# facebookresearch/DRTK

Hardware: AMD Instinct MI355X
Metric: Mpixels/sec fwd+bwd, 100k-tri @ 2048x2048, 1/2/4/8 GPU; HBM BW % (higher is better)
Workload: dtype f32; 1 GPU; 8 views/GPU x 1 GPU, 100k-tri UV-sphere head mesh (F=100352, V=50400), 2048x2048, C=16 attribute channels, transform+rasterize+render+interpolate+mask+edge_grad_estimator+loss fwd+bwd; views_per_gpu=8, triangles=100352, vertices=50400, height=2048, width=2048, channels=16, grad_reset=set_to_none, parallelism=single GPU

## Files before the change

drtk_amd/csrc/edge_grad.hip:

```cpp
#include <cstdlib>

#include "common.hpp"
#include "segscatter.hpp"

namespace drtk_amd {
namespace {

template <typename T>
struct Vec4;
template <>
struct Vec4<float> {
  using type = float4;
};
template <>
struct Vec4<double> {
  using type = double4;
};

template <typename T>
using Quad = T __attribute__((ext_vector_type(4), aligned(sizeof(T))));

template <typename T, int VEC>
struct Row {
  T v[VEC];
  T next;
};

template <typename T, int VEC>
__device__ __forceinline__ Row<T, VEC> load_row(
    const T* __restrict__ plane, int64_t row_off, int x, int W, bool x_ok, int lane) {
  Row<T, VEC> r;
  if (x_ok) {
    if constexpr (VEC == 4) {
      if (x + 4 <= W) {
        const Quad<T> q = *reinterpret_cast<const Quad<T>*>(plane + row_off + x);
        r.v[0] = q.x, r.v[1] = q.y, r.v[2] = q.z, r.v[3] = q.w;
      } else {
#pragma unroll
        for (int j = 0; j < 4; ++j) r.v[j] = x + j < W ? plane[row_off + x + j] : T(0);
      }
    } else {
      r.v[0] = plane[row_off + x];
    }
  } else {
#pragma unroll
    for (int j = 0; j < VEC; ++j) r.v[j] = T(0);
  }
  r.next = __shfl_down(r.v[0], 1);
  return r;
}

#ifndef DRTK_EDGE_SLOTS
#define DRTK_EDGE_SLOTS 64
#endif
#ifndef DRTK_ONEPASS_CAP
#define DRTK_ONEPASS_CAP 512
#endif
#ifndef DRTK_ONEPASS_WAVES
#define DRTK_ONEPASS_WAVES 6
#endif
constexpr int kOnepassCap = DRTK_ONEPASS_CAP;
#ifndef DRTK_EDGE_PRUNE
#define DRTK_EDGE_PRUNE 1
#endif

template <typename T>
struct PairArgs {
  const T* v_pix;
  const int32_t* vi;
  const T* bary_img;
  T* grad_v_pix;
  int64_t V, vi_sN;
  T M;
};

__device__ __forceinline__ int prefix4(int cnt, unsigned long long lt, int& total) {
  const unsigned long long b0 = __ballot(cnt & 1), b1 = __ballot(cnt & 2), b2 = __ballot(cnt & 4);
  total = __popcll(b0) + 2 * __popcll(b1) + 4 * __popcll(b2);
  return __popcll(b0 & lt) + 2 * __popcll(b1 & lt) + 4 * __popcll(b2 & lt);
}

template <typename T, int AXIS, int SLOTS>
__device__ __forceinline__ void scatter_pair_round(
    bool act, int px, int y, T term, const int32_t* __restrict__ idx_n, const T* __restrict__ v_n,
    const int32_t* __restrict__ vi_n, const T* __restrict__ bary_n, int64_t HW, int W, T M, int32_t* keys,
    TableAcc* vals, T* __restrict__ grad_n);

template <typename T, int R>
__device__ __forceinline__ uint32_t needed_pair_flags(
    uint32_t flags, int lane, int strip_x0, int y0, const int32_t* __restrict__ idx_n, const T* __restrict__ v_n,
    const int32_t* __restrict__ vi_n, int W, uint32_t* list, uint32_t* mask);

template <typename T, int VEC, int R, int WAVES, bool SCATTER = false>
__global__ __launch_bounds__(WAVES * kWave, SCATTER ? DRTK_ONEPASS_WAVES : 1) void edge_dots_kernel(
    const T* __restrict__ img, const T* __restrict__ grad_output, const int32_t* __restrict__ index_img, int C,
    int H, int W, int strips_x, T* __restrict__ gdx, T* __restrict__ gdy, int strip, T* __restrict__ zero_out,
    int64_t zero_count, PairArgs<T> pairs) {
  static_assert(!SCATTER || (VEC == 4 && 8 * R <= 32 && sizeof(T) == 4), "the pair phase works on four-pixel lanes of float; its flags are one register");
  constexpr int kSlots = DRTK_EDGE_SLOTS;
  constexpr int kCap = kOnepassCap;
  __shared__ uint2 s_list[SCATTER ? WAVES : 1][SCATTER ? kCap : 1];
  __shared__ int32_t t_keys[SCATTER ? WAVES : 1][SCATTER ? kSlots : 1];
  __shared__ TableAcc t_vals[SCATTER ? WAVES : 1][SCATTER ? kSlots * 4 : 1];
  if (zero_out) {
    const int64_t step = int64_t(gridDim.x) * gridDim.y * blockDim.x;
    for (int64_t i = (int64_t(blockIdx.y) * gridDim.x + blockIdx.x) * blockDim.x + threadIdx.x; i < zero_count; i += step) zero_out[i] = T(0);
  }
  const int64_t HW = int64_t(H) * W;
  const int n = blockIdx.y;
  const int tile = tile_index(strip);
  const int by = tile / strips_x, sx = tile - by * strips_x;
  const int lane = threadIdx.x & (kWave - 1);
  const int y0 = (by * WAVES + threadIdx.x / kWave) * R;
  if (y0 >= H) return;
  const int x = (sx * (kWave - 1) + lane) * VEC;
  const T* img_n = img + int64_t(n) * C * HW;
  const T* go_n = grad_output + int64_t(n) * C * HW;

  bool any_fg = false;
  uint32_t flags = 0;
  {
    const int32_t* idx_n = index_img + int64_t(n) * HW;
    int32_t above[4] = {-1, -1, -1, -1};
#pragma unroll
    for (int r = 0; r <= R; ++r) {
      const int y = y0 + r;
      if (y < H) {
        bool fg = false;
        int32_t first = -1, last = -1;
        int32_t cur[4] = {-1, -1, -1, -1};
        if (x < W) {
          if constexpr (VEC == 4) {
            Quad<int32_t> q;
            if (x + 4 <= W) {
              q = *reinterpret_cast<const Quad<int32_t>*>(idx_n + int64_t(y) * W + x);
            } else {
              const int32_t* rp = idx_n + int64_t(y) * W + x;
              q.x = rp[0], q.y = x + 1 < W ? rp[1] : -1, q.z = x + 2 < W ? rp[2] : -1, q.w = -1;
            }
            fg = (q.x & q.y & q.z & q.w) != -1;
            first = q.x, last = q.w;
            cur[0] = q.x, cur[1] = q.y, cur[2] = q.z, cur[3] = q.w;
          } else {
            first = last = idx_n[int64_t(y) * W + x];
            fg = first != -1;
          }
        }
        int32_t left = __shfl_up(last, 1), right = __shfl_down(first, 1);
        if (lane == 0) left = (x >= 1 && x < W) ? idx_n[int64_t(y) * W + x - 1] : -1;
        if (lane == kWave - 1) right = (x + VEC < W) ? idx_n[int64_t(y) * W + x + VEC] : -1;
        any_fg = any_fg || fg || left != -1 || right != -1;
        if constexpr (SCATTER) {
#pragma unroll
          for (int j = 0; j < 4; ++j) {
            const bool in_x = lane != kWave - 1 && x + j < W - 1;
            if (r > 0 && in_x && above[j] != cur[j]) flags |= 1u << (4 * R + 4 * (r - 1) + j);
            const int32_t nr = j < 3 ? cur[(j + 1) & 3] : right;
            if (r < R && in_x && y < H - 1 && cur[j] != nr) flags |= 1u << (4 * r + j);
            above[j] = cur[j];
          }
        }
      }
    }
  }
  bool load_any = any_fg;
  if constexpr (SCATTER) {
    if (__ballot(flags != 0) == 0) return;
#if DRTK_EDGE_PRUNE
    {
      static_assert(2 * kCap >= (kWave - 1) * 8 * R && kSlots >= kWave, "the list's storage must hold a strip's pair positions, the keys' one word per lane");
      const int wave = __builtin_amdgcn_readfirstlane(threadIdx.x / kWave);
      flags = needed_pair_flags<T, R>(
          flags, lane, sx * (kWave - 1) * VEC, y0, index_img + int64_t(n) * HW, pairs.v_pix + int64_t(n) * pairs.V * 3,
          pairs.vi + int64_t(n) * pairs.vi_sN, W, reinterpret_cast<uint32_t*>(s_list[wave]), reinterpret_cast<uint32_t*>(t_keys[wave]));
      if (__ballot(flags != 0) == 0) return;
    }
#endif
    uint32_t h3 = 0;
#pragma unroll
    for (int r = 0; r < R; ++r) h3 |= flags & (8u << (4 * r));
    const int left_h3 = __shfl_up(static_cast<int>(h3), 1);
    load_any = flags != 0 || (lane > 0 && left_h3 != 0);
  } else {
    if (__ballot(any_fg) == 0) return;
  }
  const bool x_ok = x < W && load_any;

  T ax[R][VEC], ay[R][VEC];
#pragma unroll
  for (int r = 0; r < R; ++r)
#pragma unroll
    for (int j = 0; j < VEC; ++j) ax[r][j] = ay[r][j] = T(0);

  for (int c = 0; c < C; ++c) {
    const T* ip = img_n + int64_t(c) * HW;
    const T* gp = go_n + int64_t(c) * HW;
    Row<T, VEC> ri[R + 1], rg[R + 1];
#pragma unroll
    for (int r = 0; r <= R; ++r) {
      const bool y_ok = (y0 + r) < H;
      ri[r] = load_row<T, VEC>(ip, int64_t(y0 + r) * W, x, W, x_ok && y_ok, lane);
      rg[r] = load_row<T, VEC>(gp, int64_t(y0 + r) * W, x, W, x_ok && y_ok, lane);
    }
#pragma unroll
    for (int r = 0; r < R; ++r) {
#pragma unroll
      for (int j = 0; j < VEC; ++j) {
        const T inext = (j + 1 < VEC) ? ri[r].v[(j + 1) % VEC] : ri[r].next;
        const T gnext = (j + 1 < VEC) ? rg[r].v[(j + 1) % VEC] : rg[r].next;
        ax[r][j] += (inext - ri[r].v[j]) * (T(0.5) * (gnext + rg[r].v[j]));
        ay[r][j] += (ri[r + 1].v[j] - ri[r].v[j]) * (T(0.5) * (rg[r + 1].v[j] + rg[r].v[j]));
      }
    }
  }
  if constexpr (SCATTER) {
    const int wave = __builtin_amdgcn_readfirstlane(threadIdx.x / kWave);
    const int32_t* idx_n = index_img + int64_t(n) * HW;
    const T* v_n = pairs.v_pix + int64_t(n) * pairs.V * 3;
    const int32_t* vi_n = pairs.vi + int64_t(n) * pairs.vi_sN;
    const T* bary_n = pairs.bary_img + int64_t(n) * 3 * HW;
    T* grad_n = pairs.grad_v_pix + int64_t(n) * pairs.V * 3;
    const int strip_x0 = sx * (kWave - 1) * VEC;

    table_init<kSlots>(t_keys[wave]);
    for (int i = lane; i < kSlots * 4; i += kWave) t_vals[wave][i] = 0;

    const unsigned long long lt = (1ull << lane) - 1ull;
    int grand = 0;
#pragma unroll
    for (int g = 0; g < 2 * R; ++g) {
      int t;
      prefix4(__popc((flags >> (4 * g)) & 15u), lt, t);
      grand += t;
    }
    if (grand <= kCap) {
      int n_h = 0, n_all = 0;
#pragma unroll
      for (int axis = 0; axis < 2; ++axis) {
#pragma unroll
        for (int r = 0; r < R; ++r) {
          const uint32_t f = (flags >> (4 * R * axis + 4 * r)) & 15u;
          int t;
          int pos = n_all + prefix4(__popc(f), lt, t);
          n_all += t;
#pragma unroll
          for (int j = 0; j < 4; ++j) {
            if (f & (1u << j)) s_list[wave][pos++] = make_uint2((r << 8) | (lane * 4 + j), __builtin_bit_cast(uint32_t, axis == 0 ? ax[r][j] : ay[r][j]));
          }
        }
        if (axis == 0) n_h = n_all;
      }
      wave_lds_sync();

      for (int axis = 0; axis < 2; ++axis) {
        const int l_begin = axis == 0 ? 0 : n_h, l_end = axis == 0 ? n_h : n_all;
        for (int t0 = l_begin; t0 < l_end; t0 += kWave) {
          const int t = t0 + lane;
          const bool act = t < l_end;
          int px = 0, y = 0;
          T term = T(0);
          if (act) {
            const uint2 entry = s_list[wave][t];
            y = y0 + static_cast<int>(entry.x >> 8);
            px = strip_x0 + static_cast<int>(entry.x & 255u);
            term = __builtin_bit_cast(float, entry.y);
          }
          if (axis == 0) {
            scatter_pair_round<T, 0, kSlots>(act, px, y, term, idx_n, v_n, vi_n, bary_n, HW, W, pairs.M, t_keys[wave], t_vals[wave], grad_n);
          } else {
            scatter_pair_round<T, 1, kSlots>(act, px, y, term, idx_n, v_n, vi_n, bary_n, HW, W, pairs.M, t_keys[wave], t_vals[wave], grad_n);
          }
        }
      }
    } else {
      static_assert(2 * kCap >= kWave * 8 * R, "the list's storage must hold a strip's terms");
      uint32_t* s_terms = reinterpret_cast<uint32_t*>(s_list[wave]);
#pragma unroll
      for (int q = 0; q < 4 * R; ++q) {
        s_terms[q * kWave + lane] = __builtin_bit_cast(uint32_t, ax[q / 4][q % 4]);
        s_terms[(4 * R + q) * kWave + lane] = __builtin_bit_cast(uint32_t, ay[q / 4][q % 4]);
      }
      wave_lds_sync();
      for (int axis = 0; axis < 2; ++axis) {
#pragma unroll 1
        for (int k = 0; k < 4 * R; ++k) {
          const bool act = (flags >> (4 * R * axis + k)) & 1u;
          if (__ballot(act) == 0) continue;
          const T term = __builtin_bit_cast(float, s_terms[(4 * R * axis + k) * kWave + lane]);
          if (axis == 0) {
            scatter_pair_round<T, 0, kSlots>(act, x + (k & 3), y0 + (k >> 2), term, idx_n, v_n, vi_n, bary_n, HW, W, pairs.M, t_keys[wave], t_vals[wave], grad_n);
          } else {
            scatter_pair_round<T, 1, kSlots>(act, x + (k & 3), y0 + (k >> 2), term, idx_n, v_n, vi_n, bary_n, HW, W, pairs.M, t_keys[wave], t_vals[wave], grad_n);
          }
        }
      }
    }
    wave_lds_sync();
    table_flush<T, TableAcc, kSlots>(t_keys[wave], t_vals[wave], 4, 3, grad_n, 3, 0);
    return;
  }
  if (!x_ok || lane == kWave - 1) return;
  T* ox = gdx + int64_t(n) * HW;
  T* oy = gdy + int64_t(n) * HW;
#pragma unroll
  for (int r = 0; r < R; ++r) {
    const int y = y0 + r;
    if (y >= H) break;
    const int64_t o = int64_t(y) * W + x;
    if constexpr (VEC == 4) {
      if (x + 4 <= W) {
        *reinterpret_cast<Quad<T>*>(ox + o) = Quad<T>{ax[r][0], ax[r][1], ax[r][2], ax[r][3]};
        *reinterpret_cast<Quad<T>*>(oy + o) = Quad<T>{ay[r][0], ay[r][1], ay[r][2], ay[r][3]};
      } else {
#pragma unroll
        for (int j = 0; j < 4; ++j)
          if (x + j < W) ox[o + j] = ax[r][j], oy[o + j] = ay[r][j];
      }
    } else {
      ox[o] = ax[r][0];
      oy[o] = ay[r][0];
    }
  }
}

template <typename T>
struct TriInfo {
  T p0x, p0y, p1x, p1y;
  T v01x, v01y, v02x, v02y, v12x, v12y;
  T den;
  T nx, ny, nz;
  int32_t i0, i1, i2;
};

template <typename T>
__device__ __forceinline__ void load_tri(
    const T* __restrict__ v_n, const int32_t* __restrict__ vi_n, int32_t idx, TriInfo<T>& t) {
  t.i0 = t.i1 = t.i2 = 0;
  if (idx >= 0) {
    const int32_t* f = vi_n + int64_t(idx) * 3;
    t.i0 = f[0], t.i1 = f[1], t.i2 = f[2];
  }
  t.p0x = v_n[3 * (int64_t)t.i0 + 0];
  t.p0y = v_n[3 * (int64_t)t.i0 + 1];
  t.p1x = v_n[3 * (int64_t)t.i1 + 0];
  t.p1y = v_n[3 * (int64_t)t.i1 + 1];
  const T p2x = v_n[3 * (int64_t)t.i2 + 0], p2y = v_n[3 * (int64_t)t.i2 + 1];
  t.v01x = t.p1x - t.p0x;
  t.v01y = t.p1y - t.p0y;
  t.v02x = p2x - t.p0x;
  t.v02y = p2y - t.p0y;
  t.v12x = p2x - t.p1x;
  t.v12y = p2y - t.p1y;
  t.den = t.v01x * t.v02y - t.v01y * t.v02x;
}

template <typename T>
__device__ __forceinline__ bool pix_in_tri(const TriInfo<T>& t, int x, int y) {
  if (t.den != T(0)) {
    const T px = static_cast<T>(x), py = static_cast<T>(y);
    const T vp0x = px - t.p0x, vp0y = py - t.p0y;
    const T vp1x = px - t.p1x, vp1y = py - t.p1y;
    T b0 = vp1y * t.v12x - vp1x * t.v12y;
    T b1 = vp0x * t.v02y - vp0y * t.v02x;
    T b2 = vp0y * t.v01x - vp0x * t.v01y;
    const T s = t.den > T(0) ? T(1) : (t.den < T(0) ? T(-1) : T(0));
    b0 *= s;
    b1 *= s;
    b2 *= s;
    const bool inside = (b0 >= T(0)) && (b1 >= T(0)) && (b2 >= T(0));
    const bool on0 = b0 == T(0), on1 = b1 == T(0), on2 = b2 == T(0);
    const bool pos = t.den > T(0);
    const bool tl0 = pos ? (t.v12y < T(0) || (t.v12y == T(0) && t.v12x > T(0)))
                         : (t.v12y > T(0) || (t.v12y == T(0) && t.v12x < T(0)));
    const bool tl1 = pos ? (t.v02y > T(0) || (t.v02y == T(0) && t.v02x < T(0)))
                         : (t.v02y < T(0) || (t.v02y == T(0) && t.v02x > T(0)));
    const bool tl2 = pos ? (t.v01y < T(0) || (t.v01y == T(0) && t.v01x > T(0)))
                         : (t.v01y > T(0) || (t.v01y == T(0) && t.v01x < T(0)));
    return inside && !((on0 && !tl0) || (on1 && !tl1) || (on2 && !tl2));
  }
  return false;
}

__device__ __forceinline__ float sqrt_t(float x) {
  return __builtin_sqrtf(x);
}
__device__ __forceinline__ double sqrt_t(double x) {
  return __builtin_sqrt(x);
}

template <typename T>
__device__ __forceinline__ void tri_normal(const T* __restrict__ v_n, TriInfo<T>& t) {
  const T* p0 = v_n + 3 * (int64_t)t.i0;
  const T* p1 = v_n + 3 * (int64_t)t.i1;
  const T* p2 = v_n + 3 * (int64_t)t.i2;
  const T ax = p0[0] - p2[0], ay = p0[1] - p2[1], az = p0[2] - p2[2];
  const T bx = p1[0] - p0[0], by = p1[1] - p0[1], bz = p1[2] - p0[2];
  const T cx = ay * bz - az * by;
  const T cy = az * bx - ax * bz;
  const T cz = ax * by - ay * bx;
  const T inv = T(1.0) / sqrt_t(cx * cx + cy * cy + cz * cz);
  t.nx = cx * inv;
  t.ny = cy * inv;
  t.nz = cz * inv;
}

template <typename T>
__device__ __forceinline__ void get_dp_dr(T nvx, T nvy, T nfx, T nfy, T M, T& ox, T& oy) {
  const T inv_v = T(1.0) / sqrt_t(nvx * nvx + nvy * nvy);
  const T nv_x = nvx * inv_v, nv_y = nvy * inv_v;
  const T inv_f = T(1.0) / sqrt_t(nfx * nfx + nfy * nfy);
  const T nf_x = nfx * inv_f, nf_y = nfy * inv_f;
  const T bx = -nf_y, by = nf_x;
  const T d = bx * nv_x + by * nv_y;
  T q;
  if (M > T(0)) {
    const T abs_d = d < T(0) ? -d : d;
    const T abs_bx = bx < T(0) ? -bx : bx;
    const T lim = abs_bx / M;
    const T m = abs_d < lim ? lim : abs_d;
    const T safe_d = (d >= T(0) ? T(1) : T(-1)) * epsclamp(m);
    q = bx / safe_d;
  } else {
    q = bx / epsclamp(d);
  }
  ox = q * nv_x;
  oy = q * nv_y;
}

template <typename T, int AXIS>
__device__ __forceinline__ void eval_pair(
    const T* __restrict__ v_n, TriInfo<T>& tA, TriInfo<T>& tB, int32_t idxA, int32_t idxB, int xa,
    int ya, T grad_dot, T M, T& gA, T& zA, T& gB, T& zB) {
  gA = zA = gB = zB = T(0);
  const bool a_valid = idxA >= 0, b_valid = idxB >= 0;
  const bool both = a_valid && b_valid;
  const int xb = xa + (AXIS == 0 ? 1 : 0), yb = ya + (AXIS == 1 ? 1 : 0);
// ... 124 lines not shown
  const int y = in_range ? static_cast<int>(pix0 / W) : 0;
  const int x0 = in_range ? static_cast<int>(pix0 - int64_t(y) * W) : 0;

  int32_t c[4] = {-1, -1, -1, -1}, u[4], d[4];
  if (in_range) {
    const int4 q = *reinterpret_cast<const int4*>(idx_n + pix0);
    c[0] = q.x, c[1] = q.y, c[2] = q.z, c[3] = q.w;
  }
#pragma unroll
  for (int j = 0; j < 4; ++j) u[j] = d[j] = c[j];
  if (in_range && y >= 1) {
    const int4 q = *reinterpret_cast<const int4*>(idx_n + pix0 - W);
    u[0] = q.x, u[1] = q.y, u[2] = q.z, u[3] = q.w;
  }
  if (in_range && y < H - 1) {
    const int4 q = *reinterpret_cast<const int4*>(idx_n + pix0 + W);
    d[0] = q.x, d[1] = q.y, d[2] = q.z, d[3] = q.w;
  }
  int32_t lprev = __shfl_up(c[3], 1), rnext = __shfl_down(c[0], 1);
  if (in_range && lane == 0 && x0 >= 1) lprev = idx_n[pix0 - 1];
  if (in_range && lane == kWave - 1 && x0 + 4 < W) rnext = idx_n[pix0 + 4];

  bool e[4];
  int32_t nr[4], nd[4], nl[4], nu[4];
#pragma unroll
  for (int j = 0; j < 4; ++j) {
    const int x = x0 + j;
    const bool own = in_range && (x < W - 1) && (y < H - 1);
    const bool left = in_range && (x >= 1) && (y < H - 1);
    const bool up = in_range && (y >= 1) && (x < W - 1);
    nr[j] = own ? (j < 3 ? c[(j + 1) & 3] : rnext) : c[j];
    nd[j] = own ? d[j] : c[j];
    nl[j] = left ? (j > 0 ? c[(j + 3) & 3] : lprev) : c[j];
    nu[j] = up ? u[j] : c[j];
    e[j] = c[j] != nr[j] || c[j] != nd[j] || c[j] != nl[j] || c[j] != nu[j];
  }

  const V4 zero4 = V4{T(0), T(0), T(0), T(0)};
#pragma unroll
  for (int k = 0; k < 3; ++k) *reinterpret_cast<V4*>(&s_out[wave][k][lane * 4]) = zero4;
  *reinterpret_cast<int4*>(&s_nb[wave][0][lane * 4]) = make_int4(nr[0], nr[1], nr[2], nr[3]);
  *reinterpret_cast<int4*>(&s_nb[wave][1][lane * 4]) = make_int4(nd[0], nd[1], nd[2], nd[3]);
  *reinterpret_cast<int4*>(&s_nb[wave][2][lane * 4]) = make_int4(nl[0], nl[1], nl[2], nl[3]);
  *reinterpret_cast<int4*>(&s_nb[wave][3][lane * 4]) = make_int4(nu[0], nu[1], nu[2], nu[3]);
  const unsigned long long lt = (1ull << lane) - 1ull;
  int total = 0;
#pragma unroll
  for (int j = 0; j < 4; ++j) {
    const unsigned long long m = __ballot(e[j]);
    if (e[j]) s_list[wave][total + __popcll(m & lt)] = static_cast<uint16_t>(lane * 4 + j);
    total += __popcll(m);
  }
  wave_lds_sync();

  const T* v_n = v_pix + int64_t(n) * V * 3;
  const int32_t* vi_n = vi + int64_t(n) * vi_sN;
  const T* gdx_n = gdx + int64_t(n) * HW;
  const T* gdy_n = gdy + int64_t(n) * HW;
  for (int t0 = 0; t0 < total; t0 += kWave) {
    const int t = t0 + lane;
    if (t < total) {
      const int local = s_list[wave][t];
      const int64_t pix = wave_pix0 + local;
      const int py = static_cast<int>(pix / W);
      const int px = static_cast<int>(pix - int64_t(py) * W);
      const int32_t ic = idx_n[pix];
      T ox, oy, oz;
      edge_pixel<T>(
          v_n, vi_n, gdx_n, gdy_n, pix, px, py, W, ic, s_nb[wave][0][local], s_nb[wave][1][local],
          s_nb[wave][2][local], s_nb[wave][3][local], M, ox, oy, oz);
      s_out[wave][0][local] = ox;
      s_out[wave][1][local] = oy;
      s_out[wave][2][local] = oz;
    }
  }
  wave_lds_sync();
  if (in_range) {
    T* o = out + int64_t(n) * 3 * HW + pix0;
#pragma unroll
    for (int k = 0; k < 3; ++k) *reinterpret_cast<V4*>(o + int64_t(k) * HW) = *reinterpret_cast<const V4*>(&s_out[wave][k][lane * 4]);
  }
}

template <typename T, int AXIS, int SLOTS>
__device__ __forceinline__ void scatter_pair_round(
    bool act, int px, int y, T term, const int32_t* __restrict__ idx_n, const T* __restrict__ v_n,
    const int32_t* __restrict__ vi_n, const T* __restrict__ bary_n, int64_t HW, int W, T M, int32_t* keys,
    TableAcc* vals, T* __restrict__ grad_n) {
  int32_t ia = -1, ib = -1;
  T ga = T(0), za = T(0), gb = T(0), zb = T(0);
  T Ba[3] = {T(0), T(0), T(0)}, Bb[3] = {T(0), T(0), T(0)};
  int32_t va[3] = {0, 0, 0}, vb[3] = {0, 0, 0};
  if (act) {
    const int64_t pa = int64_t(y) * W + px;
    const int64_t pb = AXIS == 0 ? pa + 1 : pa + W;
    ia = idx_n[pa];
    ib = idx_n[pb];
    TriInfo<T> ta, tb;
    load_tri<T>(v_n, vi_n, ia, ta);
    load_tri<T>(v_n, vi_n, ib, tb);
    T gA, zA, gB, zB;
    eval_pair<T, AXIS>(v_n, ta, tb, ia, ib, px, y, term, M, gA, zA, gB, zB);
    ga = -gA, za = -zA, gb = -gB, zb = -zB;
    va[0] = ta.i0, va[1] = ta.i1, va[2] = ta.i2;
    vb[0] = tb.i0, vb[1] = tb.i1, vb[2] = tb.i2;
    if (ia >= 0) Ba[0] = bary_n[pa], Ba[1] = bary_n[HW + pa], Ba[2] = bary_n[2 * HW + pa];
    if (ib >= 0) Bb[0] = bary_n[pb], Bb[1] = bary_n[HW + pb], Bb[2] = bary_n[2 * HW + pb];
  }
  const bool a_on = ia >= 0 && (ga != T(0) || za != T(0));
  const bool b_on = ib >= 0 && (gb != T(0) || zb != T(0));
  T g[12];
#pragma unroll
  for (int k = 0; k < 3; ++k) {
    g[2 * k + 0] = a_on ? ga * Ba[k] : T(0);
    g[2 * k + 1] = a_on ? za * Ba[k] : T(0);
    g[6 + 2 * k + 0] = b_on ? gb * Bb[k] : T(0);
    g[6 + 2 * k + 1] = b_on ? zb * Bb[k] : T(0);
  }
  const int32_t key_a = a_on ? ia : -1, key_b = b_on ? ib : -1;
  int dist;
  bool tail;
  const int32_t left_a = __shfl_up(key_a, 1), left_b = __shfl_up(key_b, 1);
  run_rows16_heads(key_a != left_a || key_b != left_b, dist, tail);
  if (__ballot(a_on || b_on) != 0) {
    run_sums_rows16<T, 12>(g, dist);
    constexpr int c_off = AXIS == 0 ? 0 : 1, c_step = AXIS == 0 ? 2 : 1;
    if (tail && a_on) table_add<T, 3, 2, SLOTS>(keys, vals, 4, va, g, grad_n, 3, c_off, c_step);
    if (tail && b_on) table_add<T, 3, 2, SLOTS>(keys, vals, 4, vb, g + 6, grad_n, 3, c_off, c_step);
  }
}

template <typename T, int R>
__device__ __forceinline__ uint32_t needed_pair_flags(
    uint32_t flags, int lane, int strip_x0, int y0, const int32_t* __restrict__ idx_n, const T* __restrict__ v_n,
    const int32_t* __restrict__ vi_n, int W, uint32_t* list, uint32_t* mask) {
  const unsigned long long lt = (1ull << lane) - 1ull;
  mask[lane] = 0;
  int n_all = 0;
#pragma unroll
  for (int g = 0; g < 2 * R; ++g) {
    const uint32_t f = (flags >> (4 * g)) & 15u;
    int t;
    int pos = n_all + prefix4(__popc(f), lt, t);
    n_all += t;
#pragma unroll
    for (int j = 0; j < 4; ++j) {
      if (f & (1u << j)) list[pos++] = static_cast<uint32_t>((lane << 5) | (4 * g + j));
    }
  }
  wave_lds_sync();
  for (int t0 = 0; t0 < n_all; t0 += kWave) {
    const int t = t0 + lane;
    if (t < n_all) {
      const uint32_t entry = list[t];
      const int bit = static_cast<int>(entry & 31u), owner = static_cast<int>(entry >> 5);
      const bool vertical = bit >= 4 * R;
      const int k = vertical ? bit - 4 * R : bit;
      const int xa = strip_x0 + owner * 4 + (k & 3), ya = y0 + (k >> 2);
      const int xb = vertical ? xa : xa + 1, yb = vertical ? ya + 1 : ya;
      const int64_t pa = int64_t(ya) * W + xa;
      const int32_t ia = idx_n[pa], ib = idx_n[vertical ? pa + W : pa + 1];
      bool need = true;
      if (ia >= 0 && ib >= 0) {
        TriInfo<T> ta, tb;
        load_tri<T>(v_n, vi_n, ia, ta);
        load_tri<T>(v_n, vi_n, ib, tb);
        const bool a_in_b = pix_in_tri(tb, xa, ya);
        const bool b_in_a = pix_in_tri(ta, xb, yb);
        need = a_in_b || b_in_a;
      }
      if (need) atomicOr(&mask[owner], 1u << bit);
    }
  }
  wave_lds_sync();
  return mask[lane];
}

#ifndef DRTK_PAIR_ROWS
#define DRTK_PAIR_ROWS 2
#endif
constexpr int kPairRows = DRTK_PAIR_ROWS;
template <typename T>
__global__ __launch_bounds__(kBlock, sizeof(T) == 4 ? 4 : 2) void edge_scatter_pairs_kernel(
    const T* __restrict__ v_pix, const int32_t* __restrict__ vi, const int32_t* __restrict__ index_img,
    const T* __restrict__ bary_img, const T* __restrict__ gdx, const T* __restrict__ gdy, int64_t V, int64_t vi_sN,
    int H, int W, int strips_x, T M, T* __restrict__ grad_v_pix, int strip) {
  constexpr int kWaves = kBlock / kWave;
  constexpr int kRows = kPairRows;
  constexpr int kCap = kWave * 4 * 2 * 2;
  __shared__ uint16_t s_list[kWaves][kCap];
  constexpr int kSlots = DRTK_EDGE_SLOTS;
  __shared__ int32_t t_keys[kWaves][kSlots];
  __shared__ TableAcc t_vals[kWaves][kSlots * 4];

  const int64_t HW = int64_t(H) * W;
  const int n = blockIdx.y;
  const int wave = threadIdx.x / kWave, lane = threadIdx.x & (kWave - 1);
  const int wg = tile_index(strip) * kWaves + wave;
  const int ry = wg / strips_x, sx = wg - ry * strips_x;
  const int y_base = ry * kRows;
  if (y_base >= H) return;
  const int x0 = (sx * kWave + lane) * 4;
  const bool in_x = x0 < W;
  const int32_t* idx_n = index_img + int64_t(n) * HW;
  const T* v_n = v_pix + int64_t(n) * V * 3;
  const int32_t* vi_n = vi + int64_t(n) * vi_sN;
  const T* gdx_n = gdx + int64_t(n) * HW;
  const T* gdy_n = gdy + int64_t(n) * HW;
  const T* bary_n = bary_img + int64_t(n) * 3 * HW;
  T* grad_n = grad_v_pix + int64_t(n) * V * 3;

  table_init<kSlots>(t_keys[wave]);
  for (int i = lane; i < kSlots * 4; i += kWave) t_vals[wave][i] = 0;

  int32_t row[kRows + 1][4];
#pragma unroll
  for (int r = 0; r <= kRows; ++r) {
    const int y = y_base + r;
    if (in_x && y < H) {
      const int32_t* rp = idx_n + int64_t(y) * W + x0;
      if (x0 + 4 <= W) {
        const Quad<int32_t> q = *reinterpret_cast<const Quad<int32_t>*>(rp);
        row[r][0] = q.x, row[r][1] = q.y, row[r][2] = q.z, row[r][3] = q.w;
      } else {
#pragma unroll
        for (int j = 0; j < 4; ++j) row[r][j] = x0 + j < W ? rp[j] : -1;
      }
    } else {
#pragma unroll
      for (int j = 0; j < 4; ++j) row[r][j] = -1;
    }
  }
  uint32_t hf[kRows], vf[kRows];
#pragma unroll
  for (int r = 0; r < kRows; ++r) {
    const int y = y_base + r;
    int32_t rnext = __shfl_down(row[r][0], 1);
    if (in_x && y < H && lane == kWave - 1 && x0 + 4 < W) rnext = idx_n[int64_t(y) * W + x0 + 4];
    hf[r] = vf[r] = 0;
#pragma unroll
    for (int j = 0; j < 4; ++j) {
      const bool own = in_x && (x0 + j < W - 1) && (y < H - 1);
      const int32_t nr = j < 3 ? row[r][(j + 1) & 3] : rnext;
      if (own && row[r][j] != nr) hf[r] |= 1u << j;
      if (own && row[r][j] != row[r + 1][j]) vf[r] |= 1u << j;
    }
  }
  const unsigned long long lt = (1ull << lane) - 1ull;

  int grand = 0;
#pragma unroll
  for (int r = 0; r < kRows; ++r) {
    int t;
    prefix4(__popc(hf[r]), lt, t);
// ... 49 lines not shown
}

#ifndef DRTK_DOTS_ROWS
#define DRTK_DOTS_ROWS 2
#endif
#ifndef DRTK_DOTS_WAVES
#define DRTK_DOTS_WAVES 4
#endif
constexpr int kStripRows = DRTK_DOTS_ROWS;
constexpr int kDotsWaves = DRTK_DOTS_WAVES;

template <typename T>
int edge_grad_backward_impl(
    const T* v_pix, const T* img, const int32_t* index_img, const int32_t* vi, const T* grad_output,
    int64_t N, int64_t V, int64_t C, int64_t vi_sN, int64_t H, int64_t W, double max_dp_dr, T* out,
    void* workspace, hipStream_t stream) {
  const int64_t HW = H * W;
  if (N * HW == 0) return DRTK_OK;
  T* gdx = static_cast<T*>(workspace);
  T* gdy = gdx + N * HW;
  const bool vec = (W % 4 == 0) && (reinterpret_cast<uintptr_t>(img) % (4 * sizeof(T)) == 0) &&
      (reinterpret_cast<uintptr_t>(grad_output) % (4 * sizeof(T)) == 0) &&
      (reinterpret_cast<uintptr_t>(workspace) % (4 * sizeof(T)) == 0) &&
      (reinterpret_cast<uintptr_t>(index_img) % 16 == 0);
  const int px_per_wave = (kWave - 1) * 4;
  const int strips_x = static_cast<int>(ceil_div(W, px_per_wave));
  const int bands_y = static_cast<int>(ceil_div(H, kStripRows * kDotsWaves));
  const dim3 gridA(static_cast<unsigned>(int64_t(strips_x) * bands_y), static_cast<unsigned>(N));
  DRTK_LAUNCH((edge_dots_kernel<T, 4, kStripRows, kDotsWaves>), gridA, dim3(kDotsWaves * kWave), 0, stream, img, grad_output, index_img, (int)C, (int)H, (int)W, strips_x, gdx, gdy, xcd_strip(int64_t(strips_x) * (16 / (kStripRows * kDotsWaves))), static_cast<T*>(nullptr), int64_t(0), PairArgs<T>{});
  DRTK_RETURN_IF_LAUNCH_FAILED();
  const bool vec_out = vec && (reinterpret_cast<uintptr_t>(index_img) % 16 == 0) &&
      (reinterpret_cast<uintptr_t>(out) % (4 * sizeof(T)) == 0);
  if (vec_out) {
    const dim3 gridB(static_cast<unsigned>(ceil_div(HW, kBlock * 4)), static_cast<unsigned>(N));
    DRTK_LAUNCH((edge_gather4_kernel<T>), gridB, dim3(kBlock), 0, stream, v_pix, vi, index_img, gdx, gdy, V, vi_sN, (int)H, (int)W, static_cast<T>(max_dp_dr), out, xcd_strip(ceil_div(16 * W, kBlock * 4)));
  } else {
    const dim3 gridB(static_cast<unsigned>(ceil_div(HW, kBlock)), static_cast<unsigned>(N));
    DRTK_LAUNCH((edge_gather_kernel<T>), gridB, dim3(kBlock), 0, stream, v_pix, vi, index_img, gdx, gdy, V, vi_sN, (int)H, (int)W, static_cast<T>(max_dp_dr), out);
  }
  DRTK_RETURN_IF_LAUNCH_FAILED();
  return DRTK_OK;
}

template <typename T>
int launch_edge_dots(const T* img, const T* grad_output, const int32_t* index_img, int64_t N, int64_t C, int64_t H, int64_t W, T* gdx, T* gdy, hipStream_t stream, T* zero_out, int64_t zero_count) {
  const int px_per_wave = (kWave - 1) * 4;
  const int strips_x = static_cast<int>(ceil_div(W, px_per_wave));
  const int bands_y = static_cast<int>(ceil_div(H, kStripRows * kDotsWaves));
  const dim3 gridA(static_cast<unsigned>(int64_t(strips_x) * bands_y), static_cast<unsigned>(N));
  DRTK_LAUNCH((edge_dots_kernel<T, 4, kStripRows, kDotsWaves>), gridA, dim3(kDotsWaves * kWave), 0, stream, img, grad_output, index_img, (int)C, (int)H, (int)W, strips_x, gdx, gdy, xcd_strip(int64_t(strips_x) * (16 / (kStripRows * kDotsWaves))), zero_out, zero_count, PairArgs<T>{});
  DRTK_RETURN_IF_LAUNCH_FAILED();
  return DRTK_OK;
}

inline bool aligned_to(const void* p, size_t a) {
  return reinterpret_cast<uintptr_t>(p) % a == 0;
}

#ifndef DRTK_EDGE_ONEPASS
#define DRTK_EDGE_ONEPASS 1
#endif
#ifndef DRTK_EDGE_ONEPASS_MIN_PX
#define DRTK_EDGE_ONEPASS_MIN_PX (int64_t(1) << 20)
#endif
inline bool edge_onepass_wanted(int64_t pixels) {
  const char* e = std::getenv("DRTK_AMD_EDGE_ONEPASS");
  if (e && e[0] && !e[1] && (e[0] == '0' || e[0] == '1')) return e[0] == '1';
  return pixels >= DRTK_EDGE_ONEPASS_MIN_PX;
}

template <typename T>
int edge_grad_backward_fused_impl(
    drtk_dtype_t dtype, const T* v_pix, const T* img, const int32_t* index_img, const int32_t* vi,
    const T* bary_img, const T* grad_output, int64_t N, int64_t V, int64_t C, int64_t F, int64_t vi_sN,
    int64_t H, int64_t W, double max_dp_dr, T* grad_v_pix, void* workspace, size_t workspace_bytes,
    hipStream_t stream) {
  const int64_t HW = H * W;
  if (N * HW == 0) {
    if (N * V > 0 && fill_bytes_async(grad_v_pix, 0, sizeof(T) * N * V * 3, stream) != DRTK_OK) return DRTK_ERR_LAUNCH;
    return DRTK_OK;
  }
#if DRTK_EDGE_ONEPASS
  if constexpr (std::is_same<T, float>::value) {
    if (edge_onepass_wanted(N * HW)) {
      if (N * V > 0 && fill_bytes_async(grad_v_pix, 0, sizeof(T) * N * V * 3, stream) != DRTK_OK) return DRTK_ERR_LAUNCH;
      const int strips_x = static_cast<int>(ceil_div(W, (kWave - 1) * 4));
      const int bands_y = static_cast<int>(ceil_div(H, kStripRows * kDotsWaves));
      const dim3 grid(static_cast<unsigned>(int64_t(strips_x) * bands_y), static_cast<unsigned>(N));
      const PairArgs<T> pairs{v_pix, vi, bary_img, grad_v_pix, V, vi_sN, static_cast<T>(max_dp_dr)};
      DRTK_LAUNCH((edge_dots_kernel<T, 4, kStripRows, kDotsWaves, true>), grid, dim3(kDotsWaves * kWave), 0, stream, img, grad_output, index_img, (int)C, (int)H, (int)W, strips_x, static_cast<T*>(nullptr), static_cast<T*>(nullptr), xcd_strip(int64_t(strips_x) * (16 / (kStripRows * kDotsWaves))), static_cast<T*>(nullptr), int64_t(0), pairs);
      DRTK_RETURN_IF_LAUNCH_FAILED();
      return DRTK_OK;
    }
  }
#endif
  T* gdx = static_cast<T*>(workspace);
  T* gdy = gdx + N * HW;
  const int st = launch_edge_dots<T>(img, grad_output, index_img, N, C, H, W, gdx, gdy, stream, grad_v_pix, N * V * 3);
  if (st != DRTK_OK) return st;
  const int strips_x = static_cast<int>(ceil_div(W, kWave * 4));
  const int64_t waves = int64_t(strips_x) * ceil_div(H, kPairRows);
  const dim3 grid(static_cast<unsigned>(ceil_div(waves, kBlock / kWave)), static_cast<unsigned>(N));
  const int strip = xcd_strip(ceil_div(int64_t(strips_x) * (16 / kPairRows), kBlock / kWave));
  DRTK_LAUNCH((edge_scatter_pairs_kernel<T>), grid, dim3(kBlock), 0, stream, v_pix, vi, index_img, bary_img, gdx, gdy, V, vi_sN, (int)H, (int)W, strips_x, static_cast<T>(max_dp_dr), grad_v_pix, strip);
  DRTK_RETURN_IF_LAUNCH_FAILED();
  return DRTK_OK;
}

}
}

using namespace drtk_amd;

extern "C" int drtk_amd_edge_grad_backward_workspace_bytes(
    drtk_dtype_t dtype, int64_t N, int64_t H, int64_t W, size_t* bytes) {
  if (!bytes || N < 0 || H < 0 || W < 0 || (dtype != DRTK_F32 && dtype != DRTK_F64)) return DRTK_ERR_INVALID_ARGUMENT;
  const size_t es = dtype == DRTK_F32 ? 4 : 8;
  const size_t b = size_t(2) * N * H * W * es;
  *bytes = b > 0 ? b : 16;
  return DRTK_OK;
}

extern "C" int drtk_amd_edge_grad_backward(
    drtk_dtype_t dtype, const void* v_pix, const void* img, const int32_t* index_img,
    const int32_t* vi, const void* grad_output, int64_t N, int64_t V, int64_t C, int64_t F,
    int64_t vi_sN, int64_t H, int64_t W, double max_dp_dr, void* grad_v_pix_img, void* workspace,
    size_t workspace_bytes, drtk_stream_t stream) {
  if (N < 0 || V < 0 || C < 0 || F < 0 || H < 0 || W < 0 ||
      (vi_sN != 0 && vi_sN != F * 3) || H * W >= (int64_t(1) << 31) || (dtype != DRTK_F32 && dtype != DRTK_F64))
    return DRTK_ERR_INVALID_ARGUMENT;
  if (reinterpret_cast<uintptr_t>(workspace) % 16 != 0) return DRTK_ERR_INVALID_ARGUMENT;
  size_t need = 0;
  if (drtk_amd_edge_grad_backward_workspace_bytes(dtype, N, H, W, &need) != DRTK_OK) return DRTK_ERR_INVALID_ARGUMENT;
  if (N * H * W > 0) {
    if (!index_img || !grad_v_pix_img || !workspace) return DRTK_ERR_INVALID_ARGUMENT;
    if ((N * V > 0 && !v_pix) || (F > 0 && !vi)) return DRTK_ERR_INVALID_ARGUMENT;
    if (C > 0 && (!img || !grad_output)) return DRTK_ERR_INVALID_ARGUMENT;
    if (workspace_bytes < need) return DRTK_ERR_WORKSPACE_TOO_SMALL;
  }
  {
    const size_t es = dtype_size(dtype);
    DRTK_FOR_VIEW_SLICES(N, n0, n, drtk_amd_edge_grad_backward(
        dtype, advance(v_pix, n0 * V * 3, es), advance(img, n0 * C * H * W, es), advance_typed(index_img, n0 * H * W),
        advance_typed(vi, n0 * vi_sN), advance(grad_output, n0 * C * H * W, es), n, V, C, F, vi_sN, H, W, max_dp_dr,
        advance(grad_v_pix_img, n0 * 3 * H * W, es), workspace, workspace_bytes, stream))
  }
  hipStream_t s = static_cast<hipStream_t>(stream);
  switch (dtype) {
    case DRTK_F32:
      return edge_grad_backward_impl<float>(static_cast<const float*>(v_pix), static_cast<const float*>(img), index_img, vi, static_cast<const float*>(grad_output), N, V, C, vi_sN, H, W, max_dp_dr, static_cast<float*>(grad_v_pix_img), workspace, s);
    case DRTK_F64:
      return edge_grad_backward_impl<double>(static_cast<const double*>(v_pix), static_cast<const double*>(img), index_img, vi, static_cast<const double*>(grad_output), N, V, C, vi_sN, H, W, max_dp_dr, static_cast<double*>(grad_v_pix_img), workspace, s);
    default:
      return DRTK_ERR_INVALID_ARGUMENT;
  }
}

extern "C" int drtk_amd_edge_grad_backward_fused_workspace_bytes(
    drtk_dtype_t dtype, int64_t N, int64_t H, int64_t W, size_t* bytes) {
  if (!bytes || N < 0 || H < 0 || W < 0 || (dtype != DRTK_F32 && dtype != DRTK_F64)) return DRTK_ERR_INVALID_ARGUMENT;
  const size_t es = dtype == DRTK_F32 ? 4 : 8;
  const size_t b = size_t(2) * N * H * W * es;
  *bytes = b > 0 ? b : 16;
  return DRTK_OK;
}

extern "C" int drtk_amd_edge_grad_backward_fused(
    drtk_dtype_t dtype, const void* v_pix, const void* img, const int32_t* index_img,
    const int32_t* vi, const void* bary_img, const void* grad_output, int64_t N, int64_t V, int64_t C,
    int64_t F, int64_t vi_sN, int64_t H, int64_t W, double max_dp_dr, void* grad_v_pix,
    void* workspace, size_t workspace_bytes, drtk_stream_t stream) {
  if (N < 0 || V < 0 || C < 0 || F < 0 || H < 0 || W < 0 ||
// ... 30 lines not shown
```

Before: 7219 Mpix/s.

## Use buffer loads with bounds clamping and batched pair classification in onepass edge kernel

The onepass edge-gradient kernel now reads the index image, image and gradient planes through AMD buffer resources. Out-of-range offsets return zero, so the per-lane bounds branches go away and all rows are fetched as unconditional 128-bit loads. The pair-pruning classifier is restructured to process several list entries per lane at once (default two rounds), issuing the index, face and vertex loads in separate batches to raise memory-level parallelism. A host-side addressability check limits the path to sizes that fit 32-bit byte offsets. The trade-off is more registers, which may lower occupancy, plus reliance on buffer out-of-bounds semantics for correctness at the edges.

```diff
diff --git a/drtk_amd/csrc/edge_grad.hip b/drtk_amd/csrc/edge_grad.hip
--- a/drtk_amd/csrc/edge_grad.hip
+++ b/drtk_amd/csrc/edge_grad.hip
@@ -19,6 +19,17 @@
 
 template <typename T>
 using Quad = T __attribute__((ext_vector_type(4), aligned(sizeof(T))));
+
+using BufferRsrc = __amdgpu_buffer_rsrc_t;
+__device__ __forceinline__ BufferRsrc buffer_rsrc(const void* base, uint32_t bytes) {
+  return __builtin_amdgcn_make_buffer_rsrc(const_cast<void*>(base), 0, static_cast<int>(bytes), 0x00020000);
+}
+__device__ __forceinline__ float as_float(uint32_t bits) {
+  return __builtin_bit_cast(float, bits);
+}
+__device__ __forceinline__ int32_t buffer_load_i32(BufferRsrc r, uint32_t byte_offset) {
+  return static_cast<int32_t>(__builtin_amdgcn_raw_buffer_load_b32(r, byte_offset, 0, 0));
+}
 
 template <typename T, int VEC>
 struct Row {
@@ -70,9 +81,13 @@
   const int32_t* vi;
   const T* bary_img;
   T* grad_v_pix;
-  int64_t V, vi_sN;
+  int64_t V, vi_sN, F;
   T M;
 };
+
+#ifndef DRTK_EDGE_CLASSIFY_ROUNDS
+#define DRTK_EDGE_CLASSIFY_ROUNDS 2
+#endif
 
 __device__ __forceinline__ int prefix4(int cnt, unsigned long long lt, int& total) {
   const unsigned long long b0 = __ballot(cnt & 1), b1 = __ballot(cnt & 2), b2 = __ballot(cnt & 4);
@@ -86,10 +101,10 @@
     const int32_t* __restrict__ vi_n, const T* __restrict__ bary_n, int64_t HW, int W, T M, int32_t* keys,
     TableAcc* vals, T* __restrict__ grad_n);
 
-template <typename T, int R>
+template <typename T, int R, int P>
 __device__ __forceinline__ uint32_t needed_pair_flags(
-    uint32_t flags, int lane, int strip_x0, int y0, const int32_t* __restrict__ idx_n, const T* __restrict__ v_n,
-    const int32_t* __restrict__ vi_n, int W, uint32_t* list, uint32_t* mask);
+    uint32_t flags, int lane, int strip_x0, int y0, BufferRsrc idx_rsrc, uint32_t idx_bytes, BufferRsrc v_rsrc,
+    uint32_t v_bytes, BufferRsrc vi_rsrc, uint32_t vi_bytes, int W, uint32_t* list, uint32_t* mask);
 
 template <typename T, int VEC, int R, int WAVES, bool SCATTER = false>
 __global__ __launch_bounds__(WAVES * kWave, SCATTER ? DRTK_ONEPASS_WAVES : 1) void edge_dots_kernel(
@@ -119,16 +134,46 @@
 
   bool any_fg = false;
   uint32_t flags = 0;
-  {
+  const uint32_t plane_bytes = static_cast<uint32_t>(HW) * 4u;
+  uint32_t row_off[R + 1];
+#pragma unroll
+  for (int r = 0; r <= R; ++r) row_off[r] = (x < W && y0 + r < H) ? static_cast<uint32_t>((y0 + r) * W + x) * 4u : plane_bytes;
+  const BufferRsrc idx_rsrc = buffer_rsrc(index_img + int64_t(n) * HW, plane_bytes);
+  if constexpr (SCATTER) {
+    int32_t cur[R + 1][4];
+#pragma unroll
+    for (int r = 0; r <= R; ++r) {
+      const auto q = __builtin_amdgcn_raw_buffer_load_b128(idx_rsrc, row_off[r], 0, 0);
+#pragma unroll
+      for (int j = 0; j < 4; ++j) cur[r][j] = static_cast<int32_t>(q[j]);
+    }
+#pragma unroll
+    for (int r = 0; r <= R; ++r)
+#pragma unroll
+      for (int j = 0; j < 4; ++j) cur[r][j] = (x + j < W && y0 + r < H) ? cur[r][j] : -1;
+    int32_t right[R + 1];
+#pragma unroll
+    for (int r = 0; r < R; ++r) right[r] = __shfl_down(cur[r][0], 1);
+    right[R] = -1;
+#pragma unroll
+    for (int r = 0; r <= R; ++r) {
+      const int y = y0 + r;
+#pragma unroll
+      for (int j = 0; j < 4; ++j) {
+        const bool in_x = lane != kWave - 1 && x + j < W - 1;
+        if (r > 0 && y < H && in_x && cur[r > 0 ? r - 1 : 0][j] != cur[r][j]) flags |= 1u << (4 * R + 4 * (r - 1) + j);
+        const int32_t nr = j < 3 ? cur[r][(j + 1) & 3] : right[r];
+        if (r < R && in_x && y < H - 1 && cur[r][j] != nr) flags |= 1u << (4 * r + j);
+      }
+    }
+  } else {
     const int32_t* idx_n = index_img + int64_t(n) * HW;
-    int32_t above[4] = {-1, -1, -1, -1};
 #pragma unroll
     for (int r = 0; r <= R; ++r) {
       const int y = y0 + r;
       if (y < H) {
         bool fg = false;
         int32_t first = -1, last = -1;
-        int32_t cur[4] = {-1, -1, -1, -1};
         if (x < W) {
           if constexpr (VEC == 4) {
             Quad<int32_t> q;
@@ -140,7 +185,6 @@
             }
             fg = (q.x & q.y & q.z & q.w) != -1;
             first = q.x, last = q.w;
-            cur[0] = q.x, cur[1] = q.y, cur[2] = q.z, cur[3] = q.w;
           } else {
             first = last = idx_n[int64_t(y) * W + x];
             fg = first != -1;
@@ -150,16 +194,6 @@
         if (lane == 0) left = (x >= 1 && x < W) ? idx_n[int64_t(y) * W + x - 1] : -1;
         if (lane == kWave - 1) right = (x + VEC < W) ? idx_n[int64_t(y) * W + x + VEC] : -1;
         any_fg = any_fg || fg || left != -1 || right != -1;
-        if constexpr (SCATTER) {
-#pragma unroll
-          for (int j = 0; j < 4; ++j) {
-            const bool in_x = lane != kWave - 1 && x + j < W - 1;
-            if (r > 0 && in_x && above[j] != cur[j]) flags |= 1u << (4 * R + 4 * (r - 1) + j);
-            const int32_t nr = j < 3 ? cur[(j + 1) & 3] : right;
-            if (r < R && in_x && y < H - 1 && cur[j] != nr) flags |= 1u << (4 * r + j);
-            above[j] = cur[j];
-          }
-        }
       }
     }
   }
@@ -170,9 +204,10 @@
     {
       static_assert(2 * kCap >= (kWave - 1) * 8 * R && kSlots >= kWave, "the list's storage must hold a strip's pair positions, the keys' one word per lane");
       const int wave = __builtin_amdgcn_readfirstlane(threadIdx.x / kWave);
-      flags = needed_pair_flags<T, R>(
-          flags, lane, sx * (kWave - 1) * VEC, y0, index_img + int64_t(n) * HW, pairs.v_pix + int64_t(n) * pairs.V * 3,
-          pairs.vi + int64_t(n) * pairs.vi_sN, W, reinterpret_cast<uint32_t*>(s_list[wave]), reinterpret_cast<uint32_t*>(t_keys[wave]));
+      const uint32_t v_bytes = static_cast<uint32_t>(pairs.V) * 12u, vi_bytes = static_cast<uint32_t>(pairs.F) * 12u;
+      flags = needed_pair_flags<T, R, DRTK_EDGE_CLASSIFY_ROUNDS>(
+          flags, lane, sx * (kWave - 1) * VEC, y0, idx_rsrc, plane_bytes, buffer_rsrc(pairs.v_pix + int64_t(n) * pairs.V * 3, v_bytes), v_bytes,
+          buffer_rsrc(pairs.vi + int64_t(n) * pairs.vi_sN, vi_bytes), vi_bytes, W, reinterpret_cast<uint32_t*>(s_list[wave]), reinterpret_cast<uint32_t*>(t_keys[wave]));
       if (__ballot(flags != 0) == 0) return;
     }
 #endif
@@ -192,15 +227,42 @@
 #pragma unroll
     for (int j = 0; j < VEC; ++j) ax[r][j] = ay[r][j] = T(0);
 
+  uint32_t ch_off[R + 1];
+#pragma unroll
+  for (int r = 0; r <= R; ++r) ch_off[r] = load_any ? row_off[r] : plane_bytes;
   for (int c = 0; c < C; ++c) {
     const T* ip = img_n + int64_t(c) * HW;
     const T* gp = go_n + int64_t(c) * HW;
     Row<T, VEC> ri[R + 1], rg[R + 1];
-#pragma unroll
-    for (int r = 0; r <= R; ++r) {
-      const bool y_ok = (y0 + r) < H;
-      ri[r] = load_row<T, VEC>(ip, int64_t(y0 + r) * W, x, W, x_ok && y_ok, lane);
-      rg[r] = load_row<T, VEC>(gp, int64_t(y0 + r) * W, x, W, x_ok && y_ok, lane);
+    if constexpr (SCATTER) {
+      const BufferRsrc i_rsrc = buffer_rsrc(ip, plane_bytes), g_rsrc = buffer_rsrc(gp, plane_bytes);
+#pragma unroll
+      for (int r = 0; r <= R; ++r) {
+        const auto qi = __builtin_amdgcn_raw_buffer_load_b128(i_rsrc, ch_off[r], 0, 0);
+        const auto qg = __builtin_amdgcn_raw_buffer_load_b128(g_rsrc, ch_off[r], 0, 0);
+#pragma unroll
+        for (int j = 0; j < 4; ++j) ri[r].v[j] = as_float(qi[j]), rg[r].v[j] = as_float(qg[j]);
+      }
+#pragma unroll
+      for (int r = 0; r <= R; ++r) {
+#pragma unroll
+        for (int j = 1; j < 4; ++j) {
+          ri[r].v[j] = x + j < W ? ri[r].v[j] : T(0);
+          rg[r].v[j] = x + j < W ? rg[r].v[j] : T(0);
+        }
+      }
+#pragma unroll
+      for (int r = 0; r < R; ++r) {
+        ri[r].next = __shfl_down(ri[r].v[0], 1);
+        rg[r].next = __shfl_down(rg[r].v[0], 1);
+      }
+    } else {
+#pragma unroll
+      for (int r = 0; r <= R; ++r) {
+        const bool y_ok = (y0 + r) < H;
+        ri[r] = load_row<T, VEC>(ip, int64_t(y0 + r) * W, x, W, x_ok && y_ok, lane);
+        rg[r] = load_row<T, VEC>(gp, int64_t(y0 + r) * W, x, W, x_ok && y_ok, lane);
+      }
     }
 #pragma unroll
     for (int r = 0; r < R; ++r) {
@@ -333,18 +395,11 @@
 };
 
 template <typename T>
-__device__ __forceinline__ void load_tri(
-    const T* __restrict__ v_n, const int32_t* __restrict__ vi_n, int32_t idx, TriInfo<T>& t) {
-  t.i0 = t.i1 = t.i2 = 0;
-  if (idx >= 0) {
-    const int32_t* f = vi_n + int64_t(idx) * 3;
-    t.i0 = f[0], t.i1 = f[1], t.i2 = f[2];
-  }
-  t.p0x = v_n[3 * (int64_t)t.i0 + 0];
-  t.p0y = v_n[3 * (int64_t)t.i0 + 1];
-  t.p1x = v_n[3 * (int64_t)t.i1 + 0];
-  t.p1y = v_n[3 * (int64_t)t.i1 + 1];
-  const T p2x = v_n[3 * (int64_t)t.i2 + 0], p2y = v_n[3 * (int64_t)t.i2 + 1];
+__device__ __forceinline__ void tri_setup(TriInfo<T>& t, T p0x, T p0y, T p1x, T p1y, T p2x, T p2y) {
+  t.p0x = p0x;
+  t.p0y = p0y;
+  t.p1x = p1x;
+  t.p1y = p1y;
   t.v01x = t.p1x - t.p0x;
   t.v01y = t.p1y - t.p0y;
   t.v02x = p2x - t.p0x;
@@ -352,6 +407,20 @@
   t.v12x = p2x - t.p1x;
   t.v12y = p2y - t.p1y;
   t.den = t.v01x * t.v02y - t.v01y * t.v02x;
+}
+
+template <typename T>
+__device__ __forceinline__ void load_tri(
+    const T* __restrict__ v_n, const int32_t* __restrict__ vi_n, int32_t idx, TriInfo<T>& t) {
+  t.i0 = t.i1 = t.i2 = 0;
+  if (idx >= 0) {
+    const int32_t* f = vi_n + int64_t(idx) * 3;
+    t.i0 = f[0], t.i1 = f[1], t.i2 = f[2];
+  }
+  const T p0x = v_n[3 * (int64_t)t.i0 + 0], p0y = v_n[3 * (int64_t)t.i0 + 1];
+  const T p1x = v_n[3 * (int64_t)t.i1 + 0], p1y = v_n[3 * (int64_t)t.i1 + 1];
+  const T p2x = v_n[3 * (int64_t)t.i2 + 0], p2y = v_n[3 * (int64_t)t.i2 + 1];
+  tri_setup<T>(t, p0x, p0y, p1x, p1y, p2x, p2y);
 }
 
 template <typename T>
@@ -642,6 +711,9 @@
   }
 }
 
+#ifndef DRTK_EDGE_BARY_EARLY
+#define DRTK_EDGE_BARY_EARLY 0
+#endif
 template <typename T, int AXIS, int SLOTS>
 __device__ __forceinline__ void scatter_pair_round(
     bool act, int px, int y, T term, const int32_t* __restrict__ idx_n, const T* __restrict__ v_n,
@@ -656,6 +728,9 @@
     const int64_t pb = AXIS == 0 ? pa + 1 : pa + W;
     ia = idx_n[pa];
     ib = idx_n[pb];
+#if DRTK_EDGE_BARY_EARLY
+    const T ea[3] = {bary_n[pa], bary_n[HW + pa], bary_n[2 * HW + pa]}, eb[3] = {bary_n[pb], bary_n[HW + pb], bary_n[2 * HW + pb]};
+#endif
     TriInfo<T> ta, tb;
     load_tri<T>(v_n, vi_n, ia, ta);
     load_tri<T>(v_n, vi_n, ib, tb);
@@ -664,8 +739,13 @@
     ga = -gA, za = -zA, gb = -gB, zb = -zB;
     va[0] = ta.i0, va[1] = ta.i1, va[2] = ta.i2;
     vb[0] = tb.i0, vb[1] = tb.i1, vb[2] = tb.i2;
+#if DRTK_EDGE_BARY_EARLY
+#pragma unroll
+    for (int k = 0; k < 3; ++k) Ba[k] = ia >= 0 ? ea[k] : T(0), Bb[k] = ib >= 0 ? eb[k] : T(0);
+#else
     if (ia >= 0) Ba[0] = bary_n[pa], Ba[1] = bary_n[HW + pa], Ba[2] = bary_n[2 * HW + pa];
     if (ib >= 0) Bb[0] = bary_n[pb], Bb[1] = bary_n[HW + pb], Bb[2] = bary_n[2 * HW + pb];
+#endif
   }
   const bool a_on = ia >= 0 && (ga != T(0) || za != T(0));
   const bool b_on = ib >= 0 && (gb != T(0) || zb != T(0));
@@ -690,10 +770,10 @@
   }
 }
 
-template <typename T, int R>
+template <typename T, int R, int P>
 __device__ __forceinline__ uint32_t needed_pair_flags(
-    uint32_t flags, int lane, int strip_x0, int y0, const int32_t* __restrict__ idx_n, const T* __restrict__ v_n,
-    const int32_t* __restrict__ vi_n, int W, uint32_t* list, uint32_t* mask) {
+    uint32_t flags, int lane, int strip_x0, int y0, BufferRsrc idx_rsrc, uint32_t idx_bytes, BufferRsrc v_rsrc,
+    uint32_t v_bytes, BufferRsrc vi_rsrc, uint32_t vi_bytes, int W, uint32_t* list, uint32_t* mask) {
   const unsigned long long lt = (1ull << lane) - 1ull;
   mask[lane] = 0;
   int n_all = 0;
@@ -709,27 +789,58 @@
     }
   }
   wave_lds_sync();
-  for (int t0 = 0; t0 < n_all; t0 += kWave) {
-    const int t = t0 + lane;
-    if (t < n_all) {
-      const uint32_t entry = list[t];
-      const int bit = static_cast<int>(entry & 31u), owner = static_cast<int>(entry >> 5);
+  for (int t0 = 0; t0 < n_all; t0 += kWave * P) {
+    bool valid[P], both[P];
+    uint32_t entry[P];
+    int xa[P], ya[P], xb[P], yb[P];
+    int32_t id[P][2], corner[P][2][3];
+    T pos[P][2][3][2];
+#pragma unroll
+    for (int p = 0; p < P; ++p) {
+      const int t = t0 + p * kWave + lane;
+      valid[p] = t < n_all;
+      entry[p] = list[valid[p] ? t : 0];
+    }
+#pragma unroll
+    for (int p = 0; p < P; ++p) {
+      const int bit = static_cast<int>(entry[p] & 31u), owner = static_cast<int>(entry[p] >> 5);
       const bool vertical = bit >= 4 * R;
       const int k = vertical ? bit - 4 * R : bit;
-      const int xa = strip_x0 + owner * 4 + (k & 3), ya = y0 + (k >> 2);
-      const int xb = vertical ? xa : xa + 1, yb = vertical ? ya + 1 : ya;
-      const int64_t pa = int64_t(ya) * W + xa;
-      const int32_t ia = idx_n[pa], ib = idx_n[vertical ? pa + W : pa + 1];
-      bool need = true;
-      if (ia >= 0 && ib >= 0) {
-        TriInfo<T> ta, tb;
-        load_tri<T>(v_n, vi_n, ia, ta);
-        load_tri<T>(v_n, vi_n, ib, tb);
-        const bool a_in_b = pix_in_tri(tb, xa, ya);
-        const bool b_in_a = pix_in_tri(ta, xb, yb);
-        need = a_in_b || b_in_a;
-      }
-      if (need) atomicOr(&mask[owner], 1u << bit);
+      xa[p] = strip_x0 + owner * 4 + (k & 3), ya[p] = y0 + (k >> 2);
+      xb[p] = vertical ? xa[p] : xa[p] + 1, yb[p] = vertical ? ya[p] + 1 : ya[p];
+      id[p][0] = buffer_load_i32(idx_rsrc, valid[p] ? static_cast<uint32_t>(ya[p] * W + xa[p]) * 4u : idx_bytes);
+      id[p][1] = buffer_load_i32(idx_rsrc, valid[p] ? static_cast<uint32_t>(yb[p] * W + xb[p]) * 4u : idx_bytes);
+    }
+#pragma unroll
+    for (int p = 0; p < P; ++p) {
+      both[p] = valid[p] && id[p][0] >= 0 && id[p][1] >= 0;
+#pragma unroll
+      for (int s = 0; s < 2; ++s) {
+        const auto f = __builtin_amdgcn_raw_buffer_load_b96(vi_rsrc, both[p] ? static_cast<uint32_t>(id[p][s]) * 12u : vi_bytes, 0, 0);
+#pragma unroll
+        for (int k = 0; k < 3; ++k) corner[p][s][k] = static_cast<int32_t>(f[k]);
+      }
+    }
+#pragma unroll
+    for (int p = 0; p < P; ++p) {
+#pragma unroll
+      for (int s = 0; s < 2; ++s) {
+#pragma unroll
+        for (int k = 0; k < 3; ++k) {
+          const auto xy = __builtin_amdgcn_raw_buffer_load_b64(v_rsrc, both[p] ? static_cast<uint32_t>(corner[p][s][k]) * 12u : v_bytes, 0, 0);
+          pos[p][s][k][0] = as_float(xy[0]), pos[p][s][k][1] = as_float(xy[1]);
+        }
+      }
+    }
+#pragma unroll
+    for (int p = 0; p < P; ++p) {
+      TriInfo<T> ta, tb;
+      tri_setup<T>(ta, pos[p][0][0][0], pos[p][0][0][1], pos[p][0][1][0], pos[p][0][1][1], pos[p][0][2][0], pos[p][0][2][1]);
+      tri_setup<T>(tb, pos[p][1][0][0], pos[p][1][0][1], pos[p][1][1][0], pos[p][1][1][1], pos[p][1][2][0], pos[p][1][2][1]);
+      const bool a_in_b = pix_in_tri(tb, xa[p], ya[p]);
+      const bool b_in_a = pix_in_tri(ta, xb[p], yb[p]);
+      const bool need = valid[p] && (!both[p] || a_in_b || b_in_a);
+      if (need) atomicOr(&mask[entry[p] >> 5], 1u << (entry[p] & 31u));
     }
   }
   wave_lds_sync();
@@ -945,12 +1056,13 @@
   }
 #if DRTK_EDGE_ONEPASS
   if constexpr (std::is_same<T, float>::value) {
-    if (edge_onepass_wanted(N * HW)) {
+    const bool addressable = HW <= (int64_t(1) << 30) - 8 && V < (int64_t(1) << 32) / 12 && F < (int64_t(1) << 32) / 12;
+    if (edge_onepass_wanted(N * HW) && addressable) {
       if (N * V > 0 && fill_bytes_async(grad_v_pix, 0, sizeof(T) * N * V * 3, stream) != DRTK_OK) return DRTK_ERR_LAUNCH;
       const int strips_x = static_cast<int>(ceil_div(W, (kWave - 1) * 4));
       const int bands_y = static_cast<int>(ceil_div(H, kStripRows * kDotsWaves));
       const dim3 grid(static_cast<unsigned>(int64_t(strips_x) * bands_y), static_cast<unsigned>(N));
-      const PairArgs<T> pairs{v_pix, vi, bary_img, grad_v_pix, V, vi_sN, static_cast<T>(max_dp_dr)};
+      const PairArgs<T> pairs{v_pix, vi, bary_img, grad_v_pix, V, vi_sN, F, static_cast<T>(max_dp_dr)};
       DRTK_LAUNCH((edge_dots_kernel<T, 4, kStripRows, kDotsWaves, true>), grid, dim3(kDotsWaves * kWave), 0, stream, img, grad_output, index_img, (int)C, (int)H, (int)W, strips_x, static_cast<T*>(nullptr), static_cast<T*>(nullptr), xcd_strip(int64_t(strips_x) * (16 / (kStripRows * kDotsWaves))), static_cast<T*>(nullptr), int64_t(0), pairs);
       DRTK_RETURN_IF_LAUNCH_FAILED();
       return DRTK_OK;
```

Result: faster. 7349 Mpix/s, median of 6 (+1.8%).
